# Bebra777228/PolGen-RVC

Hardware: AMD Instinct MI355X
Metric: real-time-factor (audio-sec/wall-sec) per GPU, 30s@16kHz RMVPE->48kHz (higher is better)
Workload: dtype f32 (conv products as 3 fp16 MFMAs of a hi/lo split, fp32 accumulate; fp32 elsewhere)

## Files before the change

include/rvcx.h:

```cpp
#ifndef RVCX_H
#define RVCX_H
#include <stdint.h>

#ifdef __cplusplus
extern "C" {
#endif

typedef struct rvcx_ctx rvcx_ctx;

typedef struct {
  const char* name;
  const void* data;
  int32_t dtype;
  int32_t ndim;
  int64_t shape[4];
} rvcx_tensor;

typedef struct {
  int32_t inter_channels, hidden_channels, filter_channels, n_heads, n_layers, kernel_size;
  int32_t n_resblocks;
  int32_t res_kernels[4];
  int32_t res_dilations[4][3];
  int32_t n_ups;
  int32_t up_rates[6], up_kernels[6];
// ... 60 lines not shown
int rvcx_weights_clone(rvcx_ctx*, rvcx_ctx* src);

int rvcx_rmvpe_f0(rvcx_ctx*, int B, const float* audio_hd, int64_t n, float thred, float f0_min,
                  float f0_max, float* f0_hd, float* hidden_hd);
int rvcx_rmvpe_frames(int64_t n);
int rvcx_rmvpe_mel(rvcx_ctx*, int B, const float* audio_hd, int64_t n, float* mel_hd);
int rvcx_fcpe_f0(rvcx_ctx*, int B, const float* audio_hd, int64_t n, float threshold, float* f0_hd,
                 float* salience_hd, float* mel_hd);
int rvcx_fcpe_frames(int64_t n);
int rvcx_get_f0_fcpe_x(rvcx_ctx*, const float* x_hd, int64_t n, int64_t p_len, const rvcx_params* p, int32_t* coarse,
                       float* f0);
int rvcx_hubert_features(rvcx_ctx*, int B, const float* wav_hd, int64_t n, int output_layer,
                         float* feats_hd);
int rvcx_hubert_frames(rvcx_ctx*, int64_t n);
int rvcx_synth_infer(rvcx_ctx*, int model_id, int B, int T, const int32_t* lens,
                     const float* phone_hd, const int32_t* pitch_hd, const float* pitchf_hd,
                     const int32_t* sid, const float* z_noise_hd, const float* src_noise_hd,
                     uint64_t seed, float* out_hd);
int rvcx_synth_infer_window(rvcx_ctx*, int model_id, int B, int T, const int32_t* lens,
                            const float* phone_hd, const int32_t* pitch_hd, const float* pitchf_hd,
                            const int32_t* sid, const float* z_noise_hd, const float* src_noise_hd,
                            uint64_t seed, int dec_skip, float* out_hd);
int rvcx_synth_dec_rf(rvcx_ctx*, int model_id);
int rvcx_synth_infer_taps(rvcx_ctx*, int model_id, int B, int T, const int32_t* lens,
                          const float* phone_hd, const int32_t* pitch_hd, const float* pitchf_hd,
                          const int32_t* sid, const float* z_noise_hd, const float* src_noise_hd,
                          uint64_t seed, float* out_hd, float* stats_hd, float* zflow_hd);
int rvcx_synth_infer_head(rvcx_ctx*, int model_id, int B, int T, const int32_t* lens, const float* phone_hd,
                          const int32_t* pitch_hd, const float* pitchf_hd, const int32_t* sid,
                          const float* z_noise_hd, const float* src_noise_hd, uint64_t seed, int skip_head,
                          float* out_hd, float* zflow_hd);
int rvcx_synth_upp(rvcx_ctx*, int model_id);
int rvcx_index_blend(rvcx_ctx*, float* feats_hd, int T, float index_rate, int64_t* ids_hd,
                     float* dist_hd);

int64_t rvcx_out_len(rvcx_ctx*, int model_id, int64_t n, const rvcx_params* p);
int rvcx_convert_batch(rvcx_ctx*, int model_id, int B, const float* const* wav16k_hd,
                       const int64_t* n, const rvcx_params* p, const float* const* noise_hd,
                       int16_t* const* out_hd, float* const* out_f32_hd, int64_t* out_n);
int rvcx_convert_batch_f64(rvcx_ctx*, int model_id, int B, const double* const* wav16k_hd,
                           const int64_t* n, const rvcx_params* p, const float* const* noise_hd,
                           int16_t* const* out_hd, float* const* out_f32_hd, int64_t* out_n);
int rvcx_convert_batch_ex(rvcx_ctx*, int model_id, int B, const void* const* wav16k_hd, int wav_is_f64,
                          const int64_t* n, const rvcx_params* p, const float* const* noise_hd,
                          const rvcx_utt_extra* extra, int16_t* const* out_hd, float* const* out_f32_hd, int64_t* out_n);

// ... 204 lines not shown
```

polgen-rvc_amd/_lib.py:

```python
from __future__ import annotations

import ctypes as C
import os
import threading
import types
from typing import Optional, Sequence

import numpy as np

_HERE = os.path.dirname(os.path.abspath(__file__))
LIB_PATH = os.environ.get("RVCX_LIBRARY") or os.path.join(_HERE, "librvcx.so")


class RvcxError(RuntimeError):
    pass


class Tensor(C.Structure):
    _fields_ = [("name", C.c_char_p), ("data", C.c_void_p), ("dtype", C.c_int32),
                ("ndim", C.c_int32), ("shape", C.c_int64 * 4)]


class SynthCfg(C.Structure):
    _fields_ = [("inter_channels", C.c_int32), ("hidden_channels", C.c_int32),
# ... 87 lines not shown

def sola_reference(y, b, Lb, Lx, Ls, offset=None):
    y, b = np.asarray(y, np.float64), np.asarray(b, np.float64)
    Lb, Lx, Ls = int(Lb), int(Lx), int(Ls)
    assert y.shape == (Lb + Lx + Ls,) and b.shape == (Lx,)
    win = np.lib.stride_tricks.sliding_window_view(y[:Ls + Lx], Lx)
    den = np.sqrt((win * win).sum(1) + 1e-8)
    scores = (win @ b) / den
    mags = (np.abs(win) @ np.abs(b)) / den
    d = int(np.argmax(scores)) if offset is None else int(offset)
    out = y[d:d + Lb].copy()
    k = min(Lx, Lb)
    fin = np.sin(0.5 * np.pi * np.arange(Lx) / max(Lx - 1, 1)) ** 2
    out[:k] = y[d:d + k] * fin[:k] + b[:k] * (1.0 - fin[:k])
    return out, y[d + Lb:d + Lb + Lx].copy(), d, scores, mags


_lib = None

SYMBOLS = [
    "rvcx_create", "rvcx_destroy", "rvcx_last_error", "rvcx_version", "rvcx_load_hubert",
    "rvcx_load_rmvpe", "rvcx_index_exhaustive", "rvcx_load_crepe", "rvcx_crepe_frames", "rvcx_crepe_predict", "rvcx_op_crepe_decode", "rvcx_get_f0_crepe_x", "rvcx_load_fcpe", "rvcx_fcpe_f0", "rvcx_fcpe_frames", "rvcx_get_f0_fcpe_x", "rvcx_op_fcpe_post", "rvcx_load_synth", "rvcx_unload_synth", "rvcx_load_index", "rvcx_load_index_ivf",
    "rvcx_weights_regions", "rvcx_weights_adopt", "rvcx_weights_clone", "rvcx_rmvpe_f0", "rvcx_rmvpe_frames", "rvcx_rmvpe_mel", "rvcx_synth_infer_taps", "rvcx_hubert_features",
    "rvcx_hubert_frames", "rvcx_synth_infer", "rvcx_synth_infer_window", "rvcx_synth_dec_rf", "rvcx_synth_upp", "rvcx_index_blend",
    "rvcx_out_len", "rvcx_convert_batch", "rvcx_convert_batch_f64", "rvcx_micro_batch", "rvcx_bucket_length", "rvcx_last_micro_batches", "rvcx_last_cuts", "rvcx_noise_len",
    "rvcx_get_f0", "rvcx_get_f0_x", "rvcx_vc", "rvcx_vc_frames", "rvcx_last_timing",
    "rvcx_flop_counter", "rvcx_fp32_reruns", "rvcx_mem_info", "rvcx_conv_profile", "rvcx_conv_profile_csv", "rvcx_stream", "rvcx_op_conv1d", "rvcx_op_resblock_pair", "rvcx_bench_resblock_pair", "rvcx_bench_conv1d", "rvcx_conv_override", "rvcx_op_convtranspose1d",
    "rvcx_op_conv2d3x3", "rvcx_op_convblock2d", "rvcx_op_convtranspose2d", "rvcx_op_attention", "rvcx_op_layernorm_c",
    "rvcx_op_bigru", "rvcx_op_highpass", "rvcx_highpass_exact", "rvcx_convert_batch_ex", "rvcx_get_f0_x_ex", "rvcx_fp32_layers", "rvcx_fp32_pinned",
    "rvcx_gru_fallbacks", "rvcx_gru_publish_probe", "rvcx_debug_inject", "rvcx_f0_file_track", "rvcx_op_gemm_tm", "rvcx_op_layernorm_tm",
    "rvcx_resample_len", "rvcx_resample_f64", "rvcx_resample_f64_kind", "rvcx_bench_gemm", "rvcx_device_info",
    "rvcx_convert_submit", "rvcx_convert_wait", "rvcx_convert_poll", "rvcx_convert_inflight", "rvcx_ticket_lead_ms",
    "rvcx_synth_infer_head", "rvcx_op_sola", "rvcx_stream_open", "rvcx_stream_step", "rvcx_stream_reset", "rvcx_stream_close",
    "rvcx_stream_out_len", "rvcx_stream_noise_len", "rvcx_stream_frames",
    "rvcx_stream_open_io", "rvcx_stream_in_len", "rvcx_stream_delays", "rvcx_stream_resample_delay", "rvcx_stream_last_taps",
    "rvcx_stream_set", "rvcx_op_stream_resample",
    "rvcx_stream_open_fx", "rvcx_stream_out_channels", "rvcx_stream_set_fx", "rvcx_stream_last_fx_ms", "rvcx_op_stream_fx",
    "rvcx_fx_reverb_host",
    "rvcx_fx_chain", "rvcx_op_fx_highpass", "rvcx_op_fx_compressor", "rvcx_op_fx_gate", "rvcx_op_fx_reverb", "rvcx_op_fx_shelf",
    "rvcx_op_fx_chorus", "rvcx_op_fx_mix", "rvcx_fx_chunk", "rvcx_fx_last_passes", "rvcx_fx_cte", "rvcx_fx_delay",
    "rvcx_fx_coeffs", "rvcx_fx_highpass_host", "rvcx_fx_biquad_host", "rvcx_fx_follower_host", "rvcx_fx_compressor_host",
    "rvcx_fx_gate_host", "rvcx_fx_comb_host", "rvcx_fx_allpass_host", "rvcx_fx_chorus_host", "rvcx_fx_mix_host",
    "rvcx_op_groupnorm_gelu", "rvcx_op_hubert_conv0", "rvcx_op_sine_source", "rvcx_op_randn", "rvcx_op_reflect_pad",
    "rvcx_op_mel_post", "rvcx_op_decode_f0", "rvcx_op_avgpool2", "rvcx_op_gru_input", "rvcx_op_upsample_protect",
    "rvcx_op_resblock3", "rvcx_flac_encode_bound", "rvcx_flac_encode_s16", "rvcx_flac_info", "rvcx_flac_decode_s32", "rvcx_flac_last_error",
]

# ... 739 lines not shown
        feats0 = None if feats0 is None else f32(feats0)
        pitchf = None if pitchf is None else f32(pitchf)
        ld_out = int(p_len) if ld_out is None else int(ld_out)
        out = np.empty((Cc, ld_out), np.float32)
        self._ck(lib().rvcx_op_upsample_protect(self._h, _p(feats), _p(feats0), _p(pitchf), Cc, int(Th), int(p_len), protect,
                                                1 if use_protect else 0, ld_in, ld_out, _p(out)), "op_upsample_protect")
        return out

    def load_synth(self, cfg_struct, state: dict) -> int:
        tbl, keep = make_table(state)
        mid = C.c_int(-1)
        self._ck(lib().rvcx_load_synth(self._h, C.byref(cfg_struct), tbl, len(tbl), C.byref(mid)), "load_synth")
        return mid.value

    def unload_synth(self, model_id: int):
        self._ck(lib().rvcx_unload_synth(self._h, int(model_id)), "unload_synth")

    def synth_upp(self, model_id: int) -> int:
        return int(lib().rvcx_synth_upp(self._h, model_id))

    def synth_dec_rf(self, model_id) -> int:
        return int(lib().rvcx_synth_dec_rf(self._h, int(model_id)))

    def synth_infer(self, model_id, phone, pitch, pitchf, lens=None, sid=None, z_noise=None, src_noise=None,
                    seed=0, taps=False, dec_skip=0, skip_head=None):
        phone, pitchf = f32(phone), f32(pitchf)
        pitch = i32(pitch)
        B, T, _ = phone.shape
        upp = self.synth_upp(model_id)
        out = np.empty((B, T * upp), np.float32)
        lens = i32(np.full(B, T) if lens is None else lens)
        sid = i32(np.zeros(B) if sid is None else sid)
        zn = None if z_noise is None else f32(z_noise)
        sn = None if src_noise is None else f32(src_noise)
        if skip_head is not None:
            if taps or dec_skip:
                raise RvcxError("synth_infer: dec_skip / taps and skip_head exclude each other")
            head = int(skip_head)
            Tk = max(T - head, 0)
            if sn is not None and sn.size != B * Tk * upp:
                raise RvcxError("synth_infer(skip_head=): src_noise must hold (T - skip_head) * upp samples per item")
            out = np.empty((B, Tk * upp), np.float32)
            zflow = None if zn is None else np.empty((B, zn.shape[1], Tk), np.float32)
            self._ck(lib().rvcx_synth_infer_head(self._h, model_id, B, T, _p(lens, C.c_int32), _p(phone),
                                                 _p(pitch, C.c_int32), _p(pitchf), _p(sid, C.c_int32), _p(zn), _p(sn),
                                                 C.c_uint64(seed), head, _p(out), _p(zflow)), "synth_infer_head")
# ... 618 lines not shown
```

polgen-rvc_amd/csrc/api_stages.hip:

```cpp
#include "api_internal.h"

using namespace rvcx;
using namespace rvcx::api;

extern "C" {

static int synth_infer_impl(rvcx_ctx* ctx, int model_id, int B, int T, const int32_t* lens, const float* phone,
                            const int32_t* pitch, const float* pitchf, const int32_t* sid, const float* z_noise,
                            const float* src_noise, uint64_t seed, float* out, float* stats, float* zflow, int dec_skip,
                            int skip_head = 0);

int rvcx_synth_infer(rvcx_ctx* ctx, int model_id, int B, int T, const int32_t* lens, const float* phone,
                     const int32_t* pitch, const float* pitchf, const int32_t* sid, const float* z_noise,
                     const float* src_noise, uint64_t seed, float* out) {
  CtxLock ctx_guard_ = lock_ctx(ctx);
  return synth_infer_impl(ctx, model_id, B, T, lens, phone, pitch, pitchf, sid, z_noise, src_noise, seed, out, nullptr,
                          nullptr, 0);
}

int rvcx_synth_infer_window(rvcx_ctx* ctx, int model_id, int B, int T, const int32_t* lens, const float* phone,
                            const int32_t* pitch, const float* pitchf, const int32_t* sid, const float* z_noise,
                            const float* src_noise, uint64_t seed, int dec_skip, float* out) {
  CtxLock ctx_guard_ = lock_ctx(ctx);
  return synth_infer_impl(ctx, model_id, B, T, lens, phone, pitch, pitchf, sid, z_noise, src_noise, seed, out, nullptr,
                          nullptr, dec_skip < 0 ? 0 : dec_skip);
}

int rvcx_synth_dec_rf(rvcx_ctx* ctx, int model_id) {
  int rf = -1;
  const int rc = api_call(ctx, false, [&](Ctx* C) { rf = get_synth(*C, model_id).dec_rf_frames; });
  return rc ? -1 : rf;
}

int rvcx_synth_infer_taps(rvcx_ctx* ctx, int model_id, int B, int T, const int32_t* lens, const float* phone,
                          const int32_t* pitch, const float* pitchf, const int32_t* sid, const float* z_noise,
                          const float* src_noise, uint64_t seed, float* out, float* stats, float* zflow) {
  CtxLock ctx_guard_ = lock_ctx(ctx);
  return synth_infer_impl(ctx, model_id, B, T, lens, phone, pitch, pitchf, sid, z_noise, src_noise, seed, out, stats,
                          zflow, 0);
}

int rvcx_synth_infer_head(rvcx_ctx* ctx, int model_id, int B, int T, const int32_t* lens, const float* phone,
                          const int32_t* pitch, const float* pitchf, const int32_t* sid, const float* z_noise,
                          const float* src_noise, uint64_t seed, int skip_head, float* out, float* zflow) {
  CtxLock ctx_guard_ = lock_ctx(ctx);
  return synth_infer_impl(ctx, model_id, B, T, lens, phone, pitch, pitchf, sid, z_noise, src_noise, seed, out, nullptr,
                          zflow, 0, skip_head);
}

static int synth_infer_impl(rvcx_ctx* ctx, int model_id, int B, int T, const int32_t* lens, const float* phone,
                            const int32_t* pitch, const float* pitchf, const int32_t* sid, const float* z_noise,
                            const float* src_noise, uint64_t seed, float* out, float* stats, float* zflow, int dec_skip,
                            int skip_head) {
  API_BEGIN(ctx)
// ... 373 lines not shown
```

polgen-rvc_amd/csrc/models.h:

```cpp
#pragma once
#include <functional>

#include "../../include/rvcx.h"
#include "ctx.h"
#include "layers.h"

namespace rvcx {

struct SynthModel {
  std::shared_ptr<WeightRegion> region = std::make_shared<WeightRegion>();
  rvcx_synth_cfg cfg{};
  int upp = 1;
  int dec_rf_frames = 0;
  ConvW emb_phone;
  const float* emb_pitch = nullptr;
  struct EncLayer {
    ConvW qkv, o, ffn1, ffn2;
    AttFlag att;
    const float *rel_k = nullptr, *rel_v = nullptr;
    const float *g1 = nullptr, *b1 = nullptr, *g2 = nullptr, *b2 = nullptr;
  };
  std::vector<EncLayer> enc;
  ConvW proj;
  struct Flow {
    ConvW pre, post, cond, in_l[3], rs_l[3];
  };
  Flow flows[4];
  ConvW conv_pre, cond, conv_post;
  const float* lin_wb = nullptr;
  struct Stage {
    ConvT1dW up;
    ConvW noise;
    int noise_stride = 1, noise_pad = 0;
    ConvW noise_dense;
    int noise_dense_cin = 0;
    int ch = 0;
    ConvW c1[4][3], c2[4][3];
  };
  std::vector<Stage> stages;
  const float* emb_g = nullptr;
};

std::unique_ptr<SynthModel> synth_load(Ctx& c, const rvcx_synth_cfg& cfg, const TensorTable& t);

struct SynthIO {
  int B = 1, T = 0;
  const int* lens_host = nullptr;
  const float* phone_ct = nullptr;
  const int* pitch = nullptr;
  const float* pitchf = nullptr;
  const int* sid_host = nullptr;
  const float* z_noise = nullptr;
  const float* src_noise = nullptr;
  float* out = nullptr;
  int dec_skip = 0;
  int skip_head = 0;
  float* stats_out = nullptr;
  float* z_out = nullptr;
  hipEvent_t ev_decoder = nullptr;
};
size_t synth_arena_bytes(const SynthModel& m, int B, int T);
void synth_forward(Ctx& c, const SynthModel& m, const SynthIO& io, hipEvent_t* stage_ev );

// ... 130 lines not shown
```

polgen-rvc_amd/csrc/ops.h:

```cpp
#pragma once
#include "common.h"

namespace rvcx {

void launch_attention(const float* q, const float* k, const float* v, float* out, int B, int H, int D, int T,
                      int ld, long in_bs, long out_bs, float scale, const float* emb_rel_k, const float* emb_rel_v, int window,
                      const int* lens, float* scratch, float* split_scratch, hipStream_t stream,
                      int* ovf = nullptr ,
                      int* ovf_layer = nullptr, int seq = 0 ,
                      bool allow_h3 = true );
size_t attention_scratch_floats(int B, int H, int T, int window);
size_t attention_split_floats(int B, int H, int T);
double attention_flops(int B, int H, int D, int T);

size_t bigru_scratch_bytes(int B);
int bigru_probe_publish();
int bigru_probe_state();
void launch_bigru(const float* gi, const float* whh, const float* bhh, float* y, int B, int T, int H,
                  void* scratch, int* err, hipStream_t stream, const int* lens = nullptr);

void launch_layernorm_c(const float* x, const float* gamma, const float* beta, float* y, int B, int C, int T,
                        float eps, const int* lens, hipStream_t s);
void launch_layernorm_tm(const float* x, long ld_x, const float* gamma, const float* beta, float* y, long ld_y, void* ys,
                         long ld_ys, long rows, int C, float eps, int* ovf, int* ovf_next, int seq, hipStream_t s);
void launch_cf_to_tm(const float* x, long x_bs, float* y, long ld_y, void* ys, long ld_ys, int B, int C, int T, int* ovf,
                     int* ovf_next, int seq, hipStream_t s);
void launch_groupnorm_gelu(const float* x, const float* gamma, const float* beta, float* y, int B, int C, int T,
                           float eps, hipStream_t s, const int* lens = nullptr);
size_t hubert_conv0_part_doubles(int B, int C, int T);
void launch_hubert_conv0_gn_gelu_split(const float* wav, long wav_bs, const float* w, int K, int stride, int Cp, const float* gamma,
                                       const float* beta, double* part, float* stats, void* y_split, int B, int C, int T,
                                       float eps, hipStream_t s, const int* lens, int* ovf, int* ovf_layer, int seq);
void launch_groupnorm_gelu_split(const float* x, const float* gamma, const float* beta, float* stats, void* y_split, int B,
                                 int C, int T, float eps, hipStream_t s, const int* lens, int* ovf, int* ovf_layer, int seq);
void launch_transpose(const float* x, float* y, int B, int R, int Cc, hipStream_t s);
void launch_embed_pitch(float* x, const float* emb, const int* pitch, int B, int C, int T, float scale,
                        float slope, const int* lens, hipStream_t s);
void launch_sample_z(const float* stats, const float* noise, float* z, int B, int C, int T, const int* lens,
                     hipStream_t s);
void launch_flip_channels(const float* x, float* y, int B, int C, int T, hipStream_t s);
void launch_wn_gate(const float* a, const float* g, int goff, int gstride, float* acts, int B, int H, int T,
                    hipStream_t s);
void launch_wn_res_skip(float* x, float* out, const float* rs, int B, int H, int T, int last, int first,
                        const int* lens, hipStream_t s);
void launch_coupling_sub(float* x, const float* m, int B, int half, int T, const int* lens, hipStream_t s);
void launch_mask(float* x, int B, int C, int T, const int* lens, hipStream_t s);
void launch_add_channel_bias(float* x, const float* g, int B, int C, int T, hipStream_t s);
void launch_sine_source(const float* f0, const float* noise, float* har, int B, int T, int upp, float sr,
                        const float* lin_wb, const int* lens, double* scratch, hipStream_t s);
void launch_randn(float* out, size_t n, uint64_t seed, uint64_t offset, hipStream_t s);

void launch_reflect_pad(const float* x, float* y, int B, int n, int p, long y_bs, hipStream_t s, const int* ns = nullptr,
                        long x_bs = 0);
int* dev_ints(Arena& A, const int* v, int n, hipStream_t s);
void set_dev_ints(int* dst, const int* v, int n, hipStream_t s);
inline int* dev_ints(Arena& A, const std::vector<int>& v, hipStream_t s) { return dev_ints(A, v.data(), (int)v.size(), s); }
std::vector<int*> dev_ints_many(Arena& A, const std::vector<std::vector<int>>& vs, hipStream_t s);
void launch_magnitude(const float* ft, float* mag, int B, int nb, int F, hipStream_t s, float eps = 0.f);
void launch_mel_post(const float* mel, float* out, int B, int nmel, int F, int Tp, const float* bn,
                     hipStream_t s, const int* fs = nullptr, const int* tps = nullptr);
void launch_log_clamp(const float* x, float* y, long n, float floor, hipStream_t s);
void launch_avgpool2(const float* x, float* y, int planes, int H, int Wp, long x_ps, long y_ps, hipStream_t s);
void launch_copy_strided(const float* x, float* y, int B, long n, long x_bs, long y_bs, hipStream_t s);
void launch_gru_input(const float* x, float* y, int B, int Cc, int T, int Wp, hipStream_t s);
void launch_decode_f0(const float* sal, float* f0, int B, int T, int ld, float thred, float f0_min, float f0_max,
                      hipStream_t s);
void launch_f0_coarse(const float* f0_in, float* f0_out, int* coarse, int n, double pitch, double f0_min,
                      double f0_max, hipStream_t s);

void launch_f0_override(const double* rep, int count, int start, float* f0, int* coarse, int n, double f0_min,
// ... 41 lines not shown
```

polgen-rvc_amd/csrc/ops.hip:

```cpp
#include <algorithm>
#include <cmath>
#include <vector>

#include "conv.h"
#include "h3_device.h"
#include "ops.h"

namespace rvcx {

__device__ __forceinline__ float wave_sum(float v) {
#pragma unroll
  for (int o = 32; o > 0; o >>= 1) v += __shfl_xor(v, o);
  return v;
}

__device__ __forceinline__ float gelu_erf(float v) {
  return 0.5f * v * (1.f + erff(v * 0.70710678118654752440f));
}

constexpr int LN_TX = 16, LN_PARTS = 16, LN_MAXC = 1024, LN_RPT = LN_MAXC / LN_PARTS;
__global__ __launch_bounds__(256) void layernorm_c_kernel(const float* __restrict__ x,
                                                          const float* __restrict__ gamma,
                                                          const float* __restrict__ beta, float* __restrict__ y,
                                                          int C, int T, float eps, const int* lens) {
// ... 426 lines not shown
}

#define EW_GRID(n) dim3((unsigned)std::min<long>(cdiv64((n), 256), 1 << 20)), dim3(256)

__global__ void embed_pitch_kernel(float* x, const float* emb, const int* pitch, int C, int T, float scale,
                                   float slope, const int* lens, long total) {
  for (long idx = blockIdx.x * 256L + threadIdx.x; idx < total; idx += (long)gridDim.x * 256) {
    const int t = idx % T;
    const long bc = idx / T;
    const int c = bc % C, b = bc / C;
    float v = (x[idx] + emb[(long)pitch[(long)b * T + t] * C + c]) * scale;
    v = v > 0.f ? v : v * slope;
    if (lens && t >= lens[b]) v = 0.f;
    x[idx] = v;
  }
}
void launch_embed_pitch(float* x, const float* emb, const int* pitch, int B, int C, int T, float scale,
                        float slope, const int* lens, hipStream_t s) {
  long n = (long)B * C * T;
  hipLaunchKernelGGL(embed_pitch_kernel, EW_GRID(n), 0, s, x, emb, pitch, C, T, scale, slope, lens, n);
}

__global__ void sample_z_kernel(const float* stats, const float* noise, float* z, int C, int T, const int* lens,
                                long total) {
  for (long idx = blockIdx.x * 256L + threadIdx.x; idx < total; idx += (long)gridDim.x * 256) {
    const int t = idx % T;
    const long bc = idx / T;
    const int c = bc % C, b = bc / C;
    const float m = stats[((long)b * 2 * C + c) * T + t];
    const float logs = stats[((long)b * 2 * C + C + c) * T + t];
    float v = m + expf(logs) * noise[idx] * 0.66666f;
    if (lens && t >= lens[b]) v = 0.f;
    z[idx] = v;
  }
}
void launch_sample_z(const float* stats, const float* noise, float* z, int B, int C, int T, const int* lens,
                     hipStream_t s) {
  long n = (long)B * C * T;
  hipLaunchKernelGGL(sample_z_kernel, EW_GRID(n), 0, s, stats, noise, z, C, T, lens, n);
}

__global__ void flip_channels_kernel(const float* x, float* y, int C, int T, long total) {
  for (long idx = blockIdx.x * 256L + threadIdx.x; idx < total; idx += (long)gridDim.x * 256) {
    const int t = idx % T;
    const long bc = idx / T;
    const int c = bc % C;
    const long b = bc / C;
    y[idx] = x[(b * C + (C - 1 - c)) * T + t];
  }
}
void launch_flip_channels(const float* x, float* y, int B, int C, int T, hipStream_t s) {
  long n = (long)B * C * T;
  hipLaunchKernelGGL(flip_channels_kernel, EW_GRID(n), 0, s, x, y, C, T, n);
}

__global__ void wn_gate_kernel(const float* a, const float* g, int goff, int gstride, float* acts, int H, int T,
                               long total) {
  for (long idx = blockIdx.x * 256L + threadIdx.x; idx < total; idx += (long)gridDim.x * 256) {
    const int t = idx % T;
    const long bc = idx / T;
    const int c = bc % H;
    const long b = bc / H;
// ... 31 lines not shown
void launch_wn_res_skip(float* x, float* out, const float* rs, int B, int H, int T, int last, int first,
                        const int* lens, hipStream_t s) {
  long n = (long)B * H * T;
  hipLaunchKernelGGL(wn_res_skip_kernel, EW_GRID(n), 0, s, x, out, rs, H, T, last, first, lens, n);
}

__global__ void coupling_sub_kernel(float* x, const float* m, int half, int T, const int* lens, long total) {
  for (long idx = blockIdx.x * 256L + threadIdx.x; idx < total; idx += (long)gridDim.x * 256) {
    const int t = idx % T;
    const long bc = idx / T;
    const int c = bc % half;
    const long b = bc / half;
    const long xi = (b * 2 * half + half + c) * T + t;
    float v = x[xi] - m[idx];
    if (lens && t >= lens[b]) v = 0.f;
    x[xi] = v;
  }
}
void launch_coupling_sub(float* x, const float* m, int B, int half, int T, const int* lens, hipStream_t s) {
  long n = (long)B * half * T;
  hipLaunchKernelGGL(coupling_sub_kernel, EW_GRID(n), 0, s, x, m, half, T, lens, n);
}

__global__ void mask_kernel(float* x, int C, int T, const int* lens, long total) {
  for (long idx = blockIdx.x * 256L + threadIdx.x; idx < total; idx += (long)gridDim.x * 256) {
    const int t = idx % T;
    const long b = idx / ((long)C * T);
    if (t >= lens[b]) x[idx] = 0.f;
  }
}
void launch_mask(float* x, int B, int C, int T, const int* lens, hipStream_t s) {
  if (!lens) return;
  long n = (long)B * C * T;
  hipLaunchKernelGGL(mask_kernel, EW_GRID(n), 0, s, x, C, T, lens, n);
}

__global__ void add_channel_bias_kernel(float* x, const float* g, int T, long total) {
  for (long idx = blockIdx.x * 256L + threadIdx.x; idx < total; idx += (long)gridDim.x * 256)
    x[idx] += g[idx / T];
}
void launch_add_channel_bias(float* x, const float* g, int B, int C, int T, hipStream_t s) {
  long n = (long)B * C * T;
  hipLaunchKernelGGL(add_channel_bias_kernel, EW_GRID(n), 0, s, x, g, T, n);
}

__global__ __launch_bounds__(64) void sine_prefix_kernel(const float* f0, double* P, float* rad_out, int T, int upp,
                                                         float sr) {
  const int b = blockIdx.x, lane = threadIdx.x;
  const int seg = (T + 63) / 64;
  const int t0 = min(lane * seg, T), t1 = min(t0 + seg, T);
  const float* f = f0 + (long)b * T;
  double acc = 0.0;
  for (int t = t0; t < t1; ++t) {
    acc += (double)fmodf(f[t] / sr, 1.0f) * upp;
    acc -= floor(acc);
  }
  double incl = acc;
#pragma unroll
  for (int d = 1; d < 64; d <<= 1) {
    const double o = __shfl_up(incl, d, 64);
    if (lane >= d) incl += o;
    incl -= floor(incl);
  }
  double run = incl - acc;
  run -= floor(run);
  for (int t = t0; t < t1; ++t) {
// ... 393 lines not shown
```

polgen-rvc_amd/csrc/synth.hip:

```cpp
#include <algorithm>
#include <cmath>
#include <cstdlib>

#include "models.h"
#include "ops.h"

namespace rvcx {

std::vector<float> wn_weight(const TensorTable& t, const std::string& p, int dim) {
  if (t.has(p + ".weight")) return t.f32(p + ".weight");
  std::string gn = p + ".parametrizations.weight.original0", vn = p + ".parametrizations.weight.original1";
  if (!t.has(gn)) {
    gn = p + ".weight_g";
    vn = p + ".weight_v";
  }
  std::vector<float> g = t.f32(gn), v = t.f32(vn);
  const auto shp = t.shape(vn);
  RVCX_CHECK(shp.size() == 3, "weight-norm tensor must be 3-D: " + p);
  const int64_t d0 = shp[0], d1 = shp[1], d2 = shp[2];
  std::vector<float> w(v.size());
  if (dim == 0) {
    RVCX_CHECK((int64_t)g.size() == d0, "weight_g shape: " + p);
    for (int64_t a = 0; a < d0; ++a) {
      double ss = 0.0;
// ... 4 lines not shown
  } else {
    RVCX_CHECK((int64_t)g.size() == d2, "weight_g shape: " + p);
    for (int64_t k = 0; k < d2; ++k) {
      double ss = 0.0;
      for (int64_t i = 0; i < d0 * d1; ++i) ss += (double)v[i * d2 + k] * v[i * d2 + k];
      const float sc = g[k] / (float)std::sqrt(ss);
      for (int64_t i = 0; i < d0 * d1; ++i) w[i * d2 + k] = v[i * d2 + k] * sc;
    }
  }
  return w;
}

static ConvW load_conv(Ctx& c, const TensorTable& t, const std::string& p, bool wn = false, bool bias = true,
                       bool h3 = true) {
  std::vector<float> w = wn ? wn_weight(t, p) : t.f32(p + ".weight");
  const auto shp = wn ? t.shape(t.has(p + ".weight") ? p + ".weight"
                                : (t.has(p + ".weight_v") ? p + ".weight_v"
                                                          : p + ".parametrizations.weight.original1"))
                      : t.shape(p + ".weight");
  const int cout = (int)shp[0], cin = (int)shp[1], k = shp.size() > 2 ? (int)shp[2] : 1;
  std::vector<float> b;
  if (bias && t.has(p + ".bias")) b = t.f32(p + ".bias");
  return make_conv(c, w.data(), b.empty() ? nullptr : b.data(), cout, cin, k, 1, h3);
}

std::unique_ptr<SynthModel> synth_load(Ctx& c, const rvcx_synth_cfg& cfg, const TensorTable& t) {
  auto M = std::make_unique<SynthModel>();
  RegionScope scope(c, *M->region);
  M->cfg = cfg;
  M->upp = 1;
  for (int i = 0; i < cfg.n_ups; ++i) M->upp *= cfg.up_rates[i];
  const int hid = cfg.hidden_channels;
  RVCX_CHECK(cfg.n_resblocks <= 4 && cfg.n_ups <= 6, "synth cfg out of range");
  M->emb_phone = load_conv(c, t, "enc_p.emb_phone");
  M->emb_pitch = c.slab.upload(t.f32("enc_p.emb_pitch.weight"));
  for (int i = 0; i < cfg.n_layers; ++i) {
    SynthModel::EncLayer L;
    const std::string a = "enc_p.encoder.attn_layers." + std::to_string(i);
    std::vector<float> w, b;
    for (const char* n : {".conv_q", ".conv_k", ".conv_v"}) {
      auto wi = t.f32(a + n + ".weight");
      auto bi = t.f32(a + n + ".bias");
      w.insert(w.end(), wi.begin(), wi.end());
      b.insert(b.end(), bi.begin(), bi.end());
    }
    L.qkv = make_conv(c, w.data(), b.data(), 3 * hid, hid, 1, 1);
// ... 51 lines not shown
      const int sp = (sf0 + 15) / 16 * 16, kn = 2 * sf0, half = sf0 / 2;
      std::vector<float> w2((size_t)co * sp * 3, 0.f);
      for (int o = 0; o < co; ++o)
        for (int c2 = 0; c2 < sf0; ++c2)
          for (int m2 = 0; m2 < 3; ++m2) {
            const int j = sf0 * (m2 - 1) + c2 + half;
            if (j >= 0 && j < kn) w2[((size_t)o * sp + c2) * 3 + m2] = w1[(size_t)o * kn + j];
          }
      S.noise_dense = make_conv(c, w2.data(), b1.data(), co, sp, 3, 1, true);
      S.noise_dense_cin = sp;
    }
    S.ch = co;
    for (int j = 0; j < cfg.n_resblocks; ++j)
      for (int m = 0; m < 3; ++m) {
        const std::string rp = "dec.resblocks." + std::to_string(i * cfg.n_resblocks + j);
        S.c1[j][m] = load_conv(c, t, rp + ".convs1." + std::to_string(m), true, true, true);
        S.c2[j][m] = load_conv(c, t, rp + ".convs2." + std::to_string(m), true, true, true);
      }
    M->stages.push_back(S);
    ch = co;
  }
  M->emb_g = c.slab.upload(t.f32("emb_g.weight"));
  {
    double rf = 3.0, rate = 1.0;
    for (int i = 0; i < cfg.n_ups; ++i) {
      rf += ((cfg.up_kernels[i] - 1) / cfg.up_rates[i] + 1) / rate;
      rate *= cfg.up_rates[i];
      int res = 0;
      for (int j = 0; j < cfg.n_resblocks; ++j) {
        int r = 0;
        for (int d = 0; d < 3; ++d) r += (cfg.res_kernels[j] - 1) / 2 * (cfg.res_dilations[j][d] + 1);
        res = std::max(res, r);
      }
      rf += res / rate;
    }
    rf += 3.0 / rate;
    M->dec_rf_frames = (int)std::ceil(rf) + 2;
  }
  M->region->seal();
  return M;
}

size_t synth_arena_bytes(const SynthModel& m, int B, int T) {
  const auto& cf = m.cfg;
  size_t enc = (size_t)B * T * (size_t)(cf.input_dim + 8 * cf.hidden_channels + 2 * cf.filter_channels +
                                        4 * cf.inter_channels + 64 + (8 * 98 + 2 * 96 + 8) * cf.n_heads);
// ... 39 lines not shown
  const int head = io.skip_head, Tk = T - head;
  RVCX_CHECK(head >= 0 && Tk > 0, "synth: skip_head outside [0, T)");
  if (head > 0) {
    RVCX_CHECK(io.dec_skip == 0, "synth: dec_skip and skip_head exclude each other");
    if (io.lens_host)
      for (int b = 0; b < B; ++b) RVCX_CHECK(io.lens_host[b] == T, "synth: skip_head needs equal lengths (every item T frames)");
  }

  bool ragged = false;
  if (io.lens_host)
    for (int b = 0; b < B; ++b) ragged |= io.lens_host[b] != T;
  std::vector<const int*> lens_stage(m.stages.size() + 2, nullptr);
  const int* lens = nullptr;
  if (ragged) {
    std::vector<int> l(io.lens_host, io.lens_host + B);
    lens = upload_ints(c, l);
    lens_stage[0] = lens;
    for (size_t i = 0; i < m.stages.size(); ++i) {
      for (auto& x : l) x *= cf.up_rates[i];
      lens_stage[i + 1] = upload_ints(c, l);
    }
  }
  std::vector<int> sidv(io.sid_host, io.sid_host + B);

  const long Tupp = (long)Tk * m.upp;
  const float* pitchf = io.pitchf;
  if (head > 0) {
    float* pf = A.alloc<float>((size_t)B * Tk);
    launch_copy_strided(io.pitchf + head, pf, B, Tk, T, Tk, s);
    pitchf = pf;
  }
  float* har = A.alloc<float>((size_t)B * Tupp);
  std::vector<float*> nz(m.stages.size(), nullptr);
  std::vector<char> nz_fused(m.stages.size(), 0);
  for (size_t i = 0; i < m.stages.size(); ++i) {
    const auto& S = m.stages[i];
    ConvArgs probe = convT1d_args(S.up, nullptr, nullptr, 1, 1, cf.up_rates[i]);
    probe.pre_act = ACT_LRELU;
    probe.pre_slope = 0.1f;
    static const bool fuse_on = !getenv("RVCX_NOISE_FUSE") || atoi(getenv("RVCX_NOISE_FUSE")) != 0;
    static const int fuse_max_k = getenv("RVCX_NOISE_FUSE_K") ? atoi(getenv("RVCX_NOISE_FUSE_K")) : 4;
    nz_fused[i] = fuse_on && S.noise.cin == 1 && S.noise.groups == 1 && S.noise.k >= 1 && S.noise.cout == S.ch &&
                  S.noise.k <= fuse_max_k;
    (void)probe;
  }
  {
// ... 60 lines not shown
    a = conv1d_args(L.ffn1, x, hbuf, B, T, T, 1, 1, pl);
    a.act = ACT_RELU;
    a.lens_in = lens;
    a.lens_out = lens;
    c.conv(a);
    a = conv1d_args(L.ffn2, hbuf, tmp, B, T, T, 1, 1, pl);
    a.lens_in = lens;
    a.lens_out = lens;
    conv_set_res(a, x, hid, T);
    c.conv(a);
    launch_layernorm_c(tmp, L.g2, L.b2, x, B, hid, T, 1e-5f, nullptr, s);
  }
  float* stats = io.stats_out ? io.stats_out : A.alloc<float>((size_t)B * 2 * inter * T);
  {
    launch_mask(x, B, hid, T, lens, s);
    ConvArgs a = conv1d_args(m.proj, x, stats, B, T, T);
    a.lens_out = lens;
    c.conv(a);
  }
  tm.mark(1);

  float* z = A.alloc<float>((size_t)B * inter * T);
  float* z2 = A.alloc<float>((size_t)B * inter * T);
  launch_sample_z(stats, io.z_noise, z, B, inter, T, lens, s);
  if (head > 0) {
    launch_copy_strided(z + head, z2, B * inter, Tk, T, Tk, s);
    std::swap(z, z2);
  }
  float* g = A.alloc<float>((size_t)B * gin);
  for (int b = 0; b < B; ++b)
    RVCX_HIP(hipMemcpyAsync(g + (size_t)b * gin, m.emb_g + (size_t)sidv[b] * gin, gin * sizeof(float),
                            hipMemcpyDeviceToDevice, s));
  {
    float* h = att;
    float* xin = qkv;
    float* acts = tmp;
    float* rs = hbuf;
    RVCX_CHECK(filt >= 2 * hid, "buffer reuse assumes filter_channels >= 2*hidden");
    float* wout = A.alloc<float>((size_t)B * hid * T);
    float* mbuf = A.alloc<float>((size_t)B * half * T);
    float* gc = A.alloc<float>((size_t)B * 6 * hid);
    for (int f = 3; f >= 0; --f) {
      const auto& F = m.flows[f];
      launch_flip_channels(z, z2, B, inter, Tk, s);
      std::swap(z, z2);
      ConvArgs a = conv1d_args(F.pre, z, h, B, Tk, Tk);
      a.x_bs = (long)inter * Tk;
      a.lens_out = lens;
      c.conv(a);
      a = conv1d_args(F.cond, g, gc, B, 1, 1);
      c.conv(a);
      for (int i = 0; i < 3; ++i) {
        a = conv1d_args(F.in_l[i], h, xin, B, Tk, Tk, 1, 1, (F.in_l[i].k - 1) / 2);
        a.lens_in = lens;
        a.lens_out = lens;
        c.conv(a);
        launch_wn_gate(xin, gc, i * 2 * hid, 6 * hid, acts, B, hid, Tk, s);
        a = conv1d_args(F.rs_l[i], acts, rs, B, Tk, Tk);
        a.lens_out = lens;
        c.conv(a);
        launch_wn_res_skip(h, wout, rs, B, hid, Tk, i == 2, i == 0, lens, s);
      }
      a = conv1d_args(F.post, wout, mbuf, B, Tk, Tk);
      a.lens_out = lens;
      c.conv(a);
      launch_coupling_sub(z, mbuf, B, half, Tk, lens, s);
    }
  }
  if (io.z_out)
    RVCX_HIP(hipMemcpyAsync(io.z_out, z, (size_t)B * inter * Tk * sizeof(float), hipMemcpyDeviceToDevice, s));
  tm.mark(2);
  if (io.ev_decoder) RVCX_HIP(hipEventRecord(io.ev_decoder, s));

  if (!c.serial) RVCX_HIP(hipStreamWaitEvent(s, c.ev_src[1], 0));
  static const int dec_batch_env = getenv("RVCX_DEC_BATCH") ? std::max(1, atoi(getenv("RVCX_DEC_BATCH"))) : 8;
  bool equal_lens = true;
  if (io.lens_host)
    for (int b = 1; b < B; ++b) equal_lens &= io.lens_host[b] == io.lens_host[0];
  const int dec_batch = equal_lens ? dec_batch_env : 1;
  const int C0 = cf.up_initial_channel;
  const size_t dec_mark = A.mark();
  for (int b0 = 0; b0 < B; b0 += dec_batch) {
    const int db = std::min(dec_batch, B - b0);
    A.reset(dec_mark);
    const bool own = io.lens_host != nullptr && (db == 1 || equal_lens);
    const int Tfull = own ? io.lens_host[b0] - head : Tk;
    RVCX_CHECK(Tfull > 0 && Tfull <= Tk, "synth: item length outside (0, T]");
    const int skip = (io.dec_skip > 0 && (own || !lens) && Tfull - 2 * io.dec_skip > 2 * m.dec_rf_frames) ? io.dec_skip : 0;
    const int Td = Tfull - 2 * skip;
    float* cur = A.alloc<float>((size_t)db * C0 * Td);
    {
      ConvArgs a = conv1d_args(m.conv_pre, z + (size_t)b0 * inter * Tk + skip, cur, db, Td, Td, 1, 1, 3);
      a.x_bs = (long)inter * Tk;
      a.x_cs = Tk;
      a.lens_in = (lens && !own) ? lens + b0 : nullptr;
      c.conv(a);
      float* gcond = A.alloc<float>((size_t)db * C0);
      a = conv1d_args(m.cond, g + (size_t)b0 * gin, gcond, db, 1, 1);
      c.conv(a);
      launch_add_channel_bias(cur, gcond, db, C0, Td, s);
    }
    long Tin = Td, Tin_c = Tk, off = skip;
    for (size_t i = 0; i < m.stages.size(); ++i) {
      const auto& S = m.stages[i];
      const long Tout = Tin * cf.up_rates[i], Tout_c = Tin_c * cf.up_rates[i];
      off *= cf.up_rates[i];
      const size_t n = (size_t)db * S.ch * Tout;
      float* xs = A.alloc<float>(n);
      const size_t stage_mark = A.mark();
      float* xu = A.alloc<float>(n);
      const int nk = cf.n_resblocks;
      float* xcb[4];
      float* xtb[4];
      for (int j = 0; j < nk; ++j) {
        xcb[j] = A.alloc<float>(n);
        xtb[j] = A.alloc<float>(n);
      }
      const int* lin = (lens_stage[i] && !own) ? lens_stage[i] + b0 : nullptr;
      const int* lout = (lens_stage[i + 1] && !own) ? lens_stage[i + 1] + b0 : nullptr;
      ConvArgs a = convT1d_args(S.up, cur, xu, db, (int)Tin, (int)Tout);
      a.pre_act = ACT_LRELU;
      a.pre_slope = 0.1f;
      a.lens_in = lin;
// ... 160 lines not shown
```

Baseline: 1250.

## Precompute speaker conditioning tables and fold flips and residual adds into flow kernels

At load time the flow and decoder speaker-conditioning convolutions are precomputed for every speaker into a per-model table, with an fp32 copy and a reduced-precision copy. Inference gathers a table row instead of running the cond convs. The channel flips are folded into the sample_z and coupling_sub kernels, and the res/skip elementwise kernel is removed by having the rs conv accumulate into the h/skip buffers through its residual epilogue. This cuts several small kernel launches and memory passes per flow layer, at the cost of extra load-time work and table memory that grows with speaker count.

```diff
diff --git a/include/rvcx.h b/include/rvcx.h
--- a/include/rvcx.h
+++ b/include/rvcx.h
@@ -106,6 +106,7 @@
                             const int32_t* sid, const float* z_noise_hd, const float* src_noise_hd,
                             uint64_t seed, int dec_skip, float* out_hd);
 int rvcx_synth_dec_rf(rvcx_ctx*, int model_id);
+int rvcx_synth_cond_row(rvcx_ctx*, int model_id, int sid, int exact_fp32, float* row_h, int cap);
 int rvcx_synth_infer_taps(rvcx_ctx*, int model_id, int B, int T, const int32_t* lens,
                           const float* phone_hd, const int32_t* pitch_hd, const float* pitchf_hd,
                           const int32_t* sid, const float* z_noise_hd, const float* src_noise_hd,
diff --git a/polgen-rvc_amd/_lib.py b/polgen-rvc_amd/_lib.py
--- a/polgen-rvc_amd/_lib.py
+++ b/polgen-rvc_amd/_lib.py
@@ -133,7 +133,7 @@
     "rvcx_create", "rvcx_destroy", "rvcx_last_error", "rvcx_version", "rvcx_load_hubert",
     "rvcx_load_rmvpe", "rvcx_index_exhaustive", "rvcx_load_crepe", "rvcx_crepe_frames", "rvcx_crepe_predict", "rvcx_op_crepe_decode", "rvcx_get_f0_crepe_x", "rvcx_load_fcpe", "rvcx_fcpe_f0", "rvcx_fcpe_frames", "rvcx_get_f0_fcpe_x", "rvcx_op_fcpe_post", "rvcx_load_synth", "rvcx_unload_synth", "rvcx_load_index", "rvcx_load_index_ivf",
     "rvcx_weights_regions", "rvcx_weights_adopt", "rvcx_weights_clone", "rvcx_rmvpe_f0", "rvcx_rmvpe_frames", "rvcx_rmvpe_mel", "rvcx_synth_infer_taps", "rvcx_hubert_features",
-    "rvcx_hubert_frames", "rvcx_synth_infer", "rvcx_synth_infer_window", "rvcx_synth_dec_rf", "rvcx_synth_upp", "rvcx_index_blend",
+    "rvcx_hubert_frames", "rvcx_synth_infer", "rvcx_synth_infer_window", "rvcx_synth_dec_rf", "rvcx_synth_cond_row", "rvcx_synth_upp", "rvcx_index_blend",
     "rvcx_out_len", "rvcx_convert_batch", "rvcx_convert_batch_f64", "rvcx_micro_batch", "rvcx_bucket_length", "rvcx_last_micro_batches", "rvcx_last_cuts", "rvcx_noise_len",
     "rvcx_get_f0", "rvcx_get_f0_x", "rvcx_vc", "rvcx_vc_frames", "rvcx_last_timing",
     "rvcx_flop_counter", "rvcx_fp32_reruns", "rvcx_mem_info", "rvcx_conv_profile", "rvcx_conv_profile_csv", "rvcx_stream", "rvcx_op_conv1d", "rvcx_op_resblock_pair", "rvcx_bench_resblock_pair", "rvcx_bench_conv1d", "rvcx_conv_override", "rvcx_op_convtranspose1d",
@@ -919,6 +919,14 @@
     def synth_dec_rf(self, model_id) -> int:
         return int(lib().rvcx_synth_dec_rf(self._h, int(model_id)))
 
+    def synth_cond_row(self, model_id, sid: int, exact_fp32: bool = False) -> np.ndarray:
+        n = 1 << 16
+        row = np.empty(n, np.float32)
+        got = int(lib().rvcx_synth_cond_row(self._h, int(model_id), int(sid), 1 if exact_fp32 else 0, _p(row), n))
+        if got < 0:
+            self._ck(-1, "synth_cond_row")
+        return row[:got].copy()
+
     def synth_infer(self, model_id, phone, pitch, pitchf, lens=None, sid=None, z_noise=None, src_noise=None,
                     seed=0, taps=False, dec_skip=0, skip_head=None):
         phone, pitchf = f32(phone), f32(pitchf)
diff --git a/polgen-rvc_amd/csrc/api_stages.hip b/polgen-rvc_amd/csrc/api_stages.hip
--- a/polgen-rvc_amd/csrc/api_stages.hip
+++ b/polgen-rvc_amd/csrc/api_stages.hip
@@ -30,6 +30,20 @@
   int rf = -1;
   const int rc = api_call(ctx, false, [&](Ctx* C) { rf = get_synth(*C, model_id).dec_rf_frames; });
   return rc ? -1 : rf;
+}
+
+int rvcx_synth_cond_row(rvcx_ctx* ctx, int model_id, int sid, int exact_fp32, float* row, int cap) {
+  int n = -1;
+  const int rc = api_call(ctx, false, [&](Ctx* C) {
+    const SynthModel& M = get_synth(*C, model_id);
+    if (sid < 0 || sid >= M.n_spk) fail("synth_cond_row: speaker id outside the model's emb_g");
+    if (!row || cap < M.cond_row) fail("synth_cond_row: buffer too small");
+    RVCX_HIP(hipDeviceSynchronize());
+    RVCX_HIP(hipMemcpy(row, M.cond_tab[exact_fp32 ? 1 : 0] + (size_t)sid * M.cond_row, (size_t)M.cond_row * sizeof(float),
+                       hipMemcpyDeviceToHost));
+    n = M.cond_row;
+  });
+  return rc ? -1 : n;
 }
 
 int rvcx_synth_infer_taps(rvcx_ctx* ctx, int model_id, int B, int T, const int32_t* lens, const float* phone,
diff --git a/polgen-rvc_amd/csrc/models.h b/polgen-rvc_amd/csrc/models.h
--- a/polgen-rvc_amd/csrc/models.h
+++ b/polgen-rvc_amd/csrc/models.h
@@ -39,6 +39,8 @@
   };
   std::vector<Stage> stages;
   const float* emb_g = nullptr;
+  const float* cond_tab[2] = {nullptr, nullptr};
+  int cond_row = 0, n_spk = 0;
 };
 
 std::unique_ptr<SynthModel> synth_load(Ctx& c, const rvcx_synth_cfg& cfg, const TensorTable& t);
diff --git a/polgen-rvc_amd/csrc/ops.h b/polgen-rvc_amd/csrc/ops.h
--- a/polgen-rvc_amd/csrc/ops.h
+++ b/polgen-rvc_amd/csrc/ops.h
@@ -37,15 +37,17 @@
 void launch_embed_pitch(float* x, const float* emb, const int* pitch, int B, int C, int T, float scale,
                         float slope, const int* lens, hipStream_t s);
 void launch_sample_z(const float* stats, const float* noise, float* z, int B, int C, int T, const int* lens,
-                     hipStream_t s);
+                     hipStream_t s, int flip = 0);
 void launch_flip_channels(const float* x, float* y, int B, int C, int T, hipStream_t s);
 void launch_wn_gate(const float* a, const float* g, int goff, int gstride, float* acts, int B, int H, int T,
                     hipStream_t s);
 void launch_wn_res_skip(float* x, float* out, const float* rs, int B, int H, int T, int last, int first,
                         const int* lens, hipStream_t s);
 void launch_coupling_sub(float* x, const float* m, int B, int half, int T, const int* lens, hipStream_t s);
+void launch_coupling_sub_flip(const float* x, const float* m, float* y, int B, int half, int T, const int* lens,
+                              hipStream_t s);
 void launch_mask(float* x, int B, int C, int T, const int* lens, hipStream_t s);
-void launch_add_channel_bias(float* x, const float* g, int B, int C, int T, hipStream_t s);
+void launch_add_channel_bias(float* x, const float* g, long g_bs, int B, int C, int T, hipStream_t s);
 void launch_sine_source(const float* f0, const float* noise, float* har, int B, int T, int upp, float sr,
                         const float* lin_wb, const int* lens, double* scratch, hipStream_t s);
 void launch_randn(float* out, size_t n, uint64_t seed, uint64_t offset, hipStream_t s);
diff --git a/polgen-rvc_amd/csrc/ops.hip b/polgen-rvc_amd/csrc/ops.hip
--- a/polgen-rvc_amd/csrc/ops.hip
+++ b/polgen-rvc_amd/csrc/ops.hip
@@ -472,7 +472,7 @@
 }
 
 __global__ void sample_z_kernel(const float* stats, const float* noise, float* z, int C, int T, const int* lens,
-                                long total) {
+                                int flip, long total) {
   for (long idx = blockIdx.x * 256L + threadIdx.x; idx < total; idx += (long)gridDim.x * 256) {
     const int t = idx % T;
     const long bc = idx / T;
@@ -481,13 +481,13 @@
     const float logs = stats[((long)b * 2 * C + C + c) * T + t];
     float v = m + expf(logs) * noise[idx] * 0.66666f;
     if (lens && t >= lens[b]) v = 0.f;
-    z[idx] = v;
+    z[flip ? ((long)b * C + (C - 1 - c)) * T + t : idx] = v;
   }
 }
 void launch_sample_z(const float* stats, const float* noise, float* z, int B, int C, int T, const int* lens,
-                     hipStream_t s) {
+                     hipStream_t s, int flip) {
   long n = (long)B * C * T;
-  hipLaunchKernelGGL(sample_z_kernel, EW_GRID(n), 0, s, stats, noise, z, C, T, lens, n);
+  hipLaunchKernelGGL(sample_z_kernel, EW_GRID(n), 0, s, stats, noise, z, C, T, lens, flip, n);
 }
 
 __global__ void flip_channels_kernel(const float* x, float* y, int C, int T, long total) {
@@ -565,6 +565,28 @@
   hipLaunchKernelGGL(coupling_sub_kernel, EW_GRID(n), 0, s, x, m, half, T, lens, n);
 }
 
+__global__ void coupling_sub_flip_kernel(const float* x, const float* m, float* y, int half, int T, const int* lens,
+                                         long total) {
+  const int C = 2 * half;
+  for (long idx = blockIdx.x * 256L + threadIdx.x; idx < total; idx += (long)gridDim.x * 256) {
+    const int t = idx % T;
+    const long bc = idx / T;
+    const int c = bc % C;
+    const long b = bc / C;
+    float v = x[idx];
+    if (c >= half) {
+      v -= m[(b * half + (c - half)) * T + t];
+      if (lens && t >= lens[b]) v = 0.f;
+    }
+    y[(b * C + (C - 1 - c)) * T + t] = v;
+  }
+}
+void launch_coupling_sub_flip(const float* x, const float* m, float* y, int B, int half, int T, const int* lens,
+                              hipStream_t s) {
+  long n = (long)B * 2 * half * T;
+  hipLaunchKernelGGL(coupling_sub_flip_kernel, EW_GRID(n), 0, s, x, m, y, half, T, lens, n);
+}
+
 __global__ void mask_kernel(float* x, int C, int T, const int* lens, long total) {
   for (long idx = blockIdx.x * 256L + threadIdx.x; idx < total; idx += (long)gridDim.x * 256) {
     const int t = idx % T;
@@ -578,13 +600,15 @@
   hipLaunchKernelGGL(mask_kernel, EW_GRID(n), 0, s, x, C, T, lens, n);
 }
 
-__global__ void add_channel_bias_kernel(float* x, const float* g, int T, long total) {
-  for (long idx = blockIdx.x * 256L + threadIdx.x; idx < total; idx += (long)gridDim.x * 256)
-    x[idx] += g[idx / T];
-}
-void launch_add_channel_bias(float* x, const float* g, int B, int C, int T, hipStream_t s) {
+__global__ void add_channel_bias_kernel(float* x, const float* g, long g_bs, int C, int T, long total) {
+  for (long idx = blockIdx.x * 256L + threadIdx.x; idx < total; idx += (long)gridDim.x * 256) {
+    const long bc = idx / T;
+    x[idx] += g[(bc / C) * g_bs + bc % C];
+  }
+}
+void launch_add_channel_bias(float* x, const float* g, long g_bs, int B, int C, int T, hipStream_t s) {
   long n = (long)B * C * T;
-  hipLaunchKernelGGL(add_channel_bias_kernel, EW_GRID(n), 0, s, x, g, T, n);
+  hipLaunchKernelGGL(add_channel_bias_kernel, EW_GRID(n), 0, s, x, g, g_bs, C, T, n);
 }
 
 __global__ __launch_bounds__(64) void sine_prefix_kernel(const float* f0, double* P, float* rad_out, int T, int upp,
diff --git a/polgen-rvc_amd/csrc/synth.hip b/polgen-rvc_amd/csrc/synth.hip
--- a/polgen-rvc_amd/csrc/synth.hip
+++ b/polgen-rvc_amd/csrc/synth.hip
@@ -50,6 +50,19 @@
   std::vector<float> b;
   if (bias && t.has(p + ".bias")) b = t.f32(p + ".bias");
   return make_conv(c, w.data(), b.empty() ? nullptr : b.data(), cout, cin, k, 1, h3);
+}
+
+static void fill_cond_table(Ctx& c, const SynthModel& M, float* tab) {
+  const int gin = M.cfg.gin_channels, hid = M.cfg.hidden_channels;
+  const double flops = c.flops;
+  for (int sp = 0; sp < M.n_spk; ++sp) {
+    const float* g = M.emb_g + (size_t)sp * gin;
+    float* row = tab + (size_t)sp * M.cond_row;
+    for (int f = 0; f < 4; ++f) c.conv(conv1d_args(M.flows[f].cond, g, row + (size_t)f * 6 * hid, 1, 1, 1));
+    c.conv(conv1d_args(M.cond, g, row + (size_t)4 * 6 * hid, 1, 1, 1));
+  }
+  RVCX_HIP(hipStreamSynchronize(c.stream));
+  c.flops = flops;
 }
 
 std::unique_ptr<SynthModel> synth_load(Ctx& c, const rvcx_synth_cfg& cfg, const TensorTable& t) {
@@ -147,6 +160,37 @@
   }
   M->emb_g = c.slab.upload(t.f32("emb_g.weight"));
   {
+    const auto es = t.shape("emb_g.weight");
+    RVCX_CHECK(es.size() == 2 && es[1] == cfg.gin_channels, "emb_g.weight must be (speakers, gin_channels)");
+    M->n_spk = (int)es[0];
+    for (int f = 0; f < 4; ++f)
+      RVCX_CHECK(M->flows[f].cond.cout == 6 * hid && M->flows[f].cond.cin == cfg.gin_channels, "flow cond_layer shape");
+    RVCX_CHECK(M->cond.cout == cfg.up_initial_channel && M->cond.cin == cfg.gin_channels, "dec.cond shape");
+    M->cond_row = 4 * 6 * hid + cfg.up_initial_channel;
+    const size_t bytes = (size_t)M->n_spk * M->cond_row * sizeof(float);
+    float* tab = static_cast<float*>(c.slab.cur().reserve(bytes));
+    float* tab32 = static_cast<float*>(c.slab.cur().reserve(bytes));
+    M->cond_tab[0] = tab;
+    M->cond_tab[1] = tab32;
+    {
+      const bool saved = g_force_fp32;
+      g_force_fp32 = true;
+      fill_cond_table(c, *M, tab32);
+      g_force_fp32 = saved;
+    }
+    for (int attempt = 0;; ++attempt) {
+      fill_cond_table(c, *M, tab);
+      if (!c.take_overflow()) break;
+      int idx = -1;
+      if (attempt >= 5 || M->region->first_overflow(&idx) == 0) {
+        RVCX_HIP(hipMemcpy(tab, tab32, bytes, hipMemcpyDeviceToDevice));
+        M->region->clear_overflow();
+        break;
+      }
+      M->region->drop_flag(idx);
+    }
+  }
+  {
     double rf = 3.0, rate = 1.0;
     for (int i = 0; i < cfg.n_ups; ++i) {
       rf += ((cfg.up_kernels[i] - 1) / cfg.up_rates[i] + 1) / rate;
@@ -232,6 +276,10 @@
     }
   }
   std::vector<int> sidv(io.sid_host, io.sid_host + B);
+  for (int b = 0; b < B; ++b) RVCX_CHECK(sidv[b] >= 0 && sidv[b] < m.n_spk, "synth: speaker id outside the model's emb_g");
+  static const int fold_env = getenv("RVCX_FLOW_FOLD") ? atoi(getenv("RVCX_FLOW_FOLD")) : 3;
+  const bool fold = (fold_env & 1) != 0;
+  const bool fold_rs = (fold_env & 2) != 0;
 
   const long Tupp = (long)Tk * m.upp;
   const float* pitchf = io.pitchf;
@@ -338,49 +386,93 @@
 
   float* z = A.alloc<float>((size_t)B * inter * T);
   float* z2 = A.alloc<float>((size_t)B * inter * T);
-  launch_sample_z(stats, io.z_noise, z, B, inter, T, lens, s);
+  launch_sample_z(stats, io.z_noise, z, B, inter, T, lens, s, fold && head == 0);
   if (head > 0) {
     launch_copy_strided(z + head, z2, B * inter, Tk, T, Tk, s);
-    std::swap(z, z2);
-  }
-  float* g = A.alloc<float>((size_t)B * gin);
-  for (int b = 0; b < B; ++b)
-    RVCX_HIP(hipMemcpyAsync(g + (size_t)b * gin, m.emb_g + (size_t)sidv[b] * gin, gin * sizeof(float),
-                            hipMemcpyDeviceToDevice, s));
+    if (fold) launch_flip_channels(z2, z, B, inter, Tk, s);
+    else std::swap(z, z2);
+  }
+  const int cond_row = m.cond_row;
+  float* g = nullptr;
+  float* gtab = nullptr;
+  if (fold) {
+    const float* tab = m.cond_tab[conv_h3_enabled() ? 0 : 1];
+    gtab = A.alloc<float>((size_t)B * cond_row);
+    for (int b = 0; b < B; ++b)
+      RVCX_HIP(hipMemcpyAsync(gtab + (size_t)b * cond_row, tab + (size_t)sidv[b] * cond_row, cond_row * sizeof(float),
+                              hipMemcpyDeviceToDevice, s));
+  } else {
+    g = A.alloc<float>((size_t)B * gin);
+    for (int b = 0; b < B; ++b)
+      RVCX_HIP(hipMemcpyAsync(g + (size_t)b * gin, m.emb_g + (size_t)sidv[b] * gin, gin * sizeof(float),
+                              hipMemcpyDeviceToDevice, s));
+  }
   {
     float* h = att;
     float* xin = qkv;
     float* acts = tmp;
     float* rs = hbuf;
     RVCX_CHECK(filt >= 2 * hid, "buffer reuse assumes filter_channels >= 2*hidden");
-    float* wout = A.alloc<float>((size_t)B * hid * T);
+    float* wout = fold_rs ? nullptr : A.alloc<float>((size_t)B * hid * T);
     float* mbuf = A.alloc<float>((size_t)B * half * T);
     float* gc = A.alloc<float>((size_t)B * 6 * hid);
+    const long hw_bs = 2L * hid * Tk;
+    if (fold_rs) {
+      h = hbuf;
+      wout = hbuf + (size_t)hid * Tk;
+    }
     for (int f = 3; f >= 0; --f) {
       const auto& F = m.flows[f];
-      launch_flip_channels(z, z2, B, inter, Tk, s);
-      std::swap(z, z2);
+      if (!fold) {
+        launch_flip_channels(z, z2, B, inter, Tk, s);
+        std::swap(z, z2);
+      }
+      if (fold_rs) {
+        RVCX_HIP(hipMemset2DAsync(wout, (size_t)hw_bs * sizeof(float), 0, (size_t)hid * Tk * sizeof(float), B, s));
+      }
       ConvArgs a = conv1d_args(F.pre, z, h, B, Tk, Tk);
       a.x_bs = (long)inter * Tk;
+      if (fold_rs) a.y_bs = hw_bs;
       a.lens_out = lens;
       c.conv(a);
-      a = conv1d_args(F.cond, g, gc, B, 1, 1);
-      c.conv(a);
+      if (!fold) {
+        a = conv1d_args(F.cond, g, gc, B, 1, 1);
+        c.conv(a);
+      }
       for (int i = 0; i < 3; ++i) {
         a = conv1d_args(F.in_l[i], h, xin, B, Tk, Tk, 1, 1, (F.in_l[i].k - 1) / 2);
+        if (fold_rs) a.x_bs = hw_bs;
         a.lens_in = lens;
         a.lens_out = lens;
         c.conv(a);
-        launch_wn_gate(xin, gc, i * 2 * hid, 6 * hid, acts, B, hid, Tk, s);
+        if (fold) launch_wn_gate(xin, gtab, (f * 3 + i) * 2 * hid, cond_row, acts, B, hid, Tk, s);
+        else launch_wn_gate(xin, gc, i * 2 * hid, 6 * hid, acts, B, hid, Tk, s);
+        if (fold_rs) {
+          RVCX_CHECK(F.rs_l[i].cout == (i == 2 ? hid : 2 * hid), "res_skip layer shape");
+          a = conv1d_args(F.rs_l[i], acts, i == 2 ? wout : h, B, Tk, Tk);
+          a.y_bs = hw_bs;
+          a.res = a.y;
+          a.res_bs = hw_bs;
+          a.res_cs = Tk;
+          a.lens_out = lens;
+          c.conv(a);
+          continue;
+        }
         a = conv1d_args(F.rs_l[i], acts, rs, B, Tk, Tk);
         a.lens_out = lens;
         c.conv(a);
         launch_wn_res_skip(h, wout, rs, B, hid, Tk, i == 2, i == 0, lens, s);
       }
       a = conv1d_args(F.post, wout, mbuf, B, Tk, Tk);
+      if (fold_rs) a.x_bs = hw_bs;
       a.lens_out = lens;
       c.conv(a);
-      launch_coupling_sub(z, mbuf, B, half, Tk, lens, s);
+      if (fold && f > 0) {
+        launch_coupling_sub_flip(z, mbuf, z2, B, half, Tk, lens, s);
+        std::swap(z, z2);
+      } else {
+        launch_coupling_sub(z, mbuf, B, half, Tk, lens, s);
+      }
     }
   }
   if (io.z_out)
@@ -411,10 +503,14 @@
       a.x_cs = Tk;
       a.lens_in = (lens && !own) ? lens + b0 : nullptr;
       c.conv(a);
-      float* gcond = A.alloc<float>((size_t)db * C0);
-      a = conv1d_args(m.cond, g + (size_t)b0 * gin, gcond, db, 1, 1);
-      c.conv(a);
-      launch_add_channel_bias(cur, gcond, db, C0, Td, s);
+      if (fold) {
+        launch_add_channel_bias(cur, gtab + (size_t)b0 * cond_row + 4 * 6 * hid, cond_row, db, C0, Td, s);
+      } else {
+        float* gcond = A.alloc<float>((size_t)db * C0);
+        a = conv1d_args(m.cond, g + (size_t)b0 * gin, gcond, db, 1, 1);
+        c.conv(a);
+        launch_add_channel_bias(cur, gcond, C0, db, C0, Td, s);
+      }
     }
     long Tin = Td, Tin_c = Tk, off = skip;
     for (size_t i = 0; i < m.stages.size(); ++i) {
```

Result: no change. 1256 (median of 6 runs) (+0.5%).
